# dmjovan/NeRF-Workspaces-Explorer

Hardware: AMD Instinct MI355X
Metric: ray-samples/sec (800x800, 192 samples, 8x256 MLP) (higher is better)
Workload: dtype f16x3 (split-fp16 MFMA, fp32 accumulate)

## Files before the change

### nerf-workspaces-explorer_amd/csrc/nwe_mfma_kernels.h

```cpp
#pragma once
#include "nwe_host.h"

namespace nwe {

typedef _Float16 h8 __attribute__((ext_vector_type(8)));
typedef float f16v __attribute__((ext_vector_type(16)));

#define LDS_AS __attribute__((address_space(3)))

constexpr int kWaves = 4;
constexpr int kRaysPerWave = 32;

template <int W, int D>
struct Shape {
    static constexpr int NT = W / 32;
    static constexpr int KH = W / 16;
    static constexpr int KG = 4;
    static constexpr int KD = 2;
    static constexpr int NTV = W / 64;
    static constexpr int KV = W / 32;
    static constexpr int N_L0 = 2 * KG / kWaves;
    static constexpr int N_H = 2 * KH / kWaves;
    static constexpr int N_S = 2 * (KH + KG) / kWaves;
    static constexpr int N_V = 2 * (KH + KD) / kWaves;
    static constexpr int N_RGB = 2 * KV / kWaves;
    static constexpr int CHUNK_BYTES = N_S * kWaves * kTileBytes;
    static constexpr int N_CHUNKS = NT + D * NT + 1 + NTV + 1;
    static constexpr int N_CHUNKS_FOLDED = N_CHUNKS - NT - 1;
    static constexpr int N_DOT_ROWS = NT + 1;
    static constexpr int N_CHUNKS_NOVIEW = D * NT + 1;
    static constexpr int n_chunks(int form) { return form == kFormFolded ? N_CHUNKS_FOLDED : (form == kFormNoViewDirs ? N_CHUNKS_NOVIEW : N_CHUNKS); }
    static constexpr int n_bias_rows(int form) { return n_chunks(form) + (form == kFormFolded ? N_DOT_ROWS : 0); }
    static constexpr int LONG_PIECES = 8;
};

struct Pend {
    f16v a;
    float4 bias[4];
};

__device__ __forceinline__ float pend_value(const Pend& t, int r, float inv_scale) {
    const float4 b = t.bias[r >> 2];
    const float bb = (r & 3) == 0 ? b.x : ((r & 3) == 1 ? b.y : ((r & 3) == 2 ? b.z : b.w));
    return __builtin_fmaf(t.a[r], inv_scale, bb);
}

typedef _Float16 h2 __attribute__((ext_vector_type(2)));

template <bool X3, bool DOT = false>
__device__ __forceinline__ void finish_elem(const Pend& t, int e, float inv_scale, float lower, float& keep, h8& hi0, h8& lo0,
                                            h8& hi1, h8& lo1, const float* dotw = nullptr, float* dot = nullptr) {
    const float v = fmaxf(pend_value(t, e, inv_scale), lower);
    if (DOT) *dot = __builtin_fmaf(dotw[8 * (e >> 2) + (e & 3)], v, *dot);
    if ((e & 1) == 0) { keep = v; return; }
    const float v0 = keep, v1 = v;
    h2 hp;
    hp[0] = (_Float16)v0; hp[1] = (_Float16)v1;
    const _Float16 h0 = hp[0], h1 = hp[1];
    _Float16 l0 = (_Float16)0.f, l1 = (_Float16)0.f;
    if (X3) {
        const uint32_t hw = __builtin_bit_cast(uint32_t, hp);
        float r0, r1;
        asm("v_fma_mix_f32 %0, %1, -1.0, %2 op_sel:[0,0,0] op_sel_hi:[1,0,0]" : "=v"(r0) : "v"(hw), "v"(v0));
        asm("v_fma_mix_f32 %0, %1, -1.0, %2 op_sel:[1,0,0] op_sel_hi:[1,0,0]" : "=v"(r1) : "v"(hw), "v"(v1));
        l0 = (_Float16)r0; l1 = (_Float16)r1;
    }
    if (e < 8) { hi0[e - 1] = h0; hi0[e] = h1; lo0[e - 1] = l0; lo0[e] = l1; }
    else { hi1[e - 9] = h0; hi1[e - 8] = h1; lo1[e - 9] = l0; lo1[e - 8] = l1; }
}

struct Epi {
    float v[16];
    float r[16];
    uint32_t hp[8];
    uint32_t lp[8];
    float dw[16];
};

template <bool X3, int NKH, int NQ, bool FEEDS, uint32_t PM>
struct EpiPlan {
    static constexpr int GPK = X3 ? 3 : 1;
    static constexpr int NS = X3 ? 8 : 5;
    static constexpr int NGAPS = GPK * NQ;
    static constexpr int D0 = FEEDS ? GPK * (NKH - 2) - 1 : NGAPS - 1;
    static constexpr int D1 = FEEDS ? GPK * (NKH - 1) - 1 : NGAPS - 1;
    static constexpr bool usable(int gi) { return gi >= 1 && gi < NGAPS && !(X3 && gi % GPK == 1 && ((PM >> (gi / GPK)) & 1u)); }
    static constexpr int gap_of(int n) {
        int c = -1;
        for (int gi = 0; gi < NGAPS; ++gi)
            if (usable(gi) && ++c == n) return gi;
        return 1 << 20;
    }
    static constexpr bool fits(int ng) { return gap_of((ng >= 2 ? ng / 2 : 1) * NS - 1) <= D0 && gap_of(ng * NS - 1) <= D1; }
    static constexpr int NG = fits(4) ? 4 : (fits(2) ? 2 : (fits(1) ? 1 : 0));
    static constexpr bool STAGED = NG > 0;
    static constexpr int GS = STAGED ? 16 / NG : 16;
    static constexpr int slot_at(int gi) {
        if (!usable(gi)) return -1;
        int c = 0;
        for (int g = 0; g < gi; ++g) c += usable(g) ? 1 : 0;
        return c < NG * NS ? c : -1;
    }
};

__device__ __forceinline__ h8 pack4(uint32_t a, uint32_t b, uint32_t c, uint32_t d) {
    typedef uint32_t u4 __attribute__((ext_vector_type(4)));
    u4 t = {a, b, c, d};
    return __builtin_bit_cast(h8, t);
}

template <class P, bool X3, int G, int ST, bool DOT>
__device__ __forceinline__ void epi_stage(const Pend& t, Epi& E, float inv_scale, float lower, h8& y0h, h8& y0l, h8& y1h, h8& y1l,
                                          const float* dotw, float& dot) {
    constexpr int st = ST, e0 = G * P::GS;
    constexpr int ST_PACK = 3, ST_RES = 4, ST_PACKLO = 5, ST_PARK = X3 ? 6 : 4;
    if constexpr (DOT) {
        static_assert(P::NS - ST_PACK >= 1, "no stage left for the dot product");
        constexpr int NDS = P::NS - ST_PACK;
        if (st == 1) {
#pragma unroll
            for (int q = e0 / 4; q < (e0 + P::GS) / 4; ++q) {
                const float4 w4 = *reinterpret_cast<const float4*>(dotw + 8 * q);
                E.dw[4 * q] = w4.x; E.dw[4 * q + 1] = w4.y; E.dw[4 * q + 2] = w4.z; E.dw[4 * q + 3] = w4.w;
            }
        }
        if (st >= ST_PACK) {
#pragma unroll
            for (int e = e0; e < e0 + P::GS; ++e)
                if ((e - e0) % NDS == st - ST_PACK) {
                    dot = __builtin_fmaf(E.dw[e], E.v[e], dot);
                    asm volatile("" : "+v"(dot));
                }
        }
    }
    if (st == 0) {
#pragma unroll
        for (int e = e0; e < e0 + P::GS; ++e) {
            float a = t.a[e];
            asm volatile("" : "+v"(a));
            E.v[e] = a;
        }
    } else if (st == 1) {
#pragma unroll
        for (int e = e0; e < e0 + P::GS; ++e) {
            const float4 b = t.bias[e >> 2];
            const float bb = (e & 3) == 0 ? b.x : ((e & 3) == 1 ? b.y : ((e & 3) == 2 ? b.z : b.w));
            E.v[e] = __builtin_fmaf(E.v[e], inv_scale, bb);
        }
    } else if (st == 2) {
#pragma unroll
        for (int e = e0; e < e0 + P::GS; ++e) E.v[e] = fmaxf(E.v[e], lower);
    } else if (st == ST_PACK) {
#pragma unroll
        for (int p = e0 / 2; p < (e0 + P::GS) / 2; ++p) {
            h2 hp;
            hp[0] = (_Float16)E.v[2 * p]; hp[1] = (_Float16)E.v[2 * p + 1];
            E.hp[p] = __builtin_bit_cast(uint32_t, hp);
            if (!X3) E.lp[p] = 0u;
        }
    } else if (X3 && st == ST_RES) {
#pragma unroll
        for (int p = e0 / 2; p < (e0 + P::GS) / 2; ++p) {
            asm("v_fma_mix_f32 %0, %1, -1.0, %2 op_sel:[0,0,0] op_sel_hi:[1,0,0]" : "=v"(E.r[2 * p]) : "v"(E.hp[p]), "v"(E.v[2 * p]));
            asm("v_fma_mix_f32 %0, %1, -1.0, %2 op_sel:[1,0,0] op_sel_hi:[1,0,0]" : "=v"(E.r[2 * p + 1]) : "v"(E.hp[p]), "v"(E.v[2 * p + 1]));
        }
    } else if (X3 && st == ST_PACKLO) {
#pragma unroll
        for (int p = e0 / 2; p < (e0 + P::GS) / 2; ++p) {
            h2 lp;
            lp[0] = (_Float16)E.r[2 * p]; lp[1] = (_Float16)E.r[2 * p + 1];
            E.lp[p] = __builtin_bit_cast(uint32_t, lp);
        }
    } else if (st == ST_PARK || st == ST_PARK + 1) {
        const bool lo = st != ST_PARK;
        if (lo && !X3) return;
        const int last = e0 + P::GS - 1;
        if (last == 7 || (P::GS == 16)) {
            if (!lo) { y0h = pack4(E.hp[0], E.hp[1], E.hp[2], E.hp[3]); asm volatile("" : "+a"(y0h)); }
            else     { y0l = pack4(E.lp[0], E.lp[1], E.lp[2], E.lp[3]); asm volatile("" : "+a"(y0l)); }
        }
        if (last == 15) {
            if (!lo) { y1h = pack4(E.hp[4], E.hp[5], E.hp[6], E.hp[7]); asm volatile("" : "+a"(y1h)); }
            else     { y1l = pack4(E.lp[4], E.lp[5], E.lp[6], E.lp[7]); asm volatile("" : "+a"(y1l)); }
        }
    }
}

template <class P, bool X3, int GI, bool DOT>
__device__ __forceinline__ void epi_gap(const Pend& t, Epi& E, float inv_scale, float lower, h8& y0h, h8& y0l, h8& y1h, h8& y1l,
                                        const float* dotw, float& dot) {
    constexpr int slot = P::slot_at(GI);
    if constexpr (slot >= 0) epi_stage<P, X3, slot / P::NS, slot % P::NS, DOT>(t, E, inv_scale, lower, y0h, y0l, y1h, y1l, dotw, dot);
}

template <bool X3>
__device__ __forceinline__ void mma3(const h8& a_hi, const h8& a_lo, const h8& x_hi, const h8& x_lo, f16v& acc) {
    acc = __builtin_amdgcn_mfma_f32_32x32x16_f16(a_hi, x_hi, acc, 0, 0, 0);
    if (X3) {
        acc = __builtin_amdgcn_mfma_f32_32x32x16_f16(a_lo, x_hi, acc, 0, 0, 0);
        acc = __builtin_amdgcn_mfma_f32_32x32x16_f16(a_hi, x_lo, acc, 0, 0, 0);
    }
}

template <int CHUNK_BYTES, bool X3>
struct Walker {
    const uint8_t* stream;
    uint32_t next_tile;
    uint32_t lds_chunks;
    uint32_t lds_tail;
    const char* buf0;
    const char* tail0;
    int t3;
    uint32_t blk_dst_tail;
    int tail_first;
    const float* bias_tab;
    int chunk;
    int b;
    int wave;
    uint32_t lane_off;
    const uint8_t* blk_src;
    uint32_t blk_dst;
    bool skip_lo = false;
#ifdef NWE_STAMPS
    unsigned long long st_pre = 0, st_wait = 0, st_post = 0, st_t0 = 0;
#endif

    __device__ __forceinline__ void start(const uint8_t* s, const float* bias) {
        stream = s; bias_tab = bias; next_tile = 0; chunk = 0; b = 0; t3 = 0;
    }
    __device__ __forceinline__ const char* cur() const { return buf0 + b * CHUNK_BYTES; }
    __device__ __forceinline__ const char* next() const { return buf0 + (b ^ 1) * CHUNK_BYTES; }
    __device__ __forceinline__ const char* tail() const { return tail0 + t3 * (2 * kTileBytes); }
    __device__ __forceinline__ void begin(int n_per_wave, int buffer, int ahead) {
        blk_src = stream + ((size_t)next_tile + (size_t)wave * n_per_wave) * kTileBytes;
        blk_dst = lds_chunks + buffer * CHUNK_BYTES + wave * n_per_wave * kTileBytes;
        next_tile += n_per_wave * kWaves;
        skip_lo = !X3 && (n_per_wave & 1) == 0;
        if (X3) {
            int slot = t3 + ahead;
            slot = slot >= 3 ? slot - 3 : slot;
            const bool lng = n_per_wave >= 8;
            tail_first = (lng && wave == kWaves - 1) ? n_per_wave - 2 : (1 << 20);
            blk_dst_tail = lds_tail + slot * (2 * kTileBytes) - (n_per_wave - 2) * kTileBytes;
        }
    }
    __device__ __forceinline__ void piece(int i, int tail_piece = -1) {
#ifdef NWE_EXP_NODMA
        return;
#endif
        if (!X3 && skip_lo && (i & 1)) return;
        const uint8_t* src = blk_src + (size_t)(i >> 2) * (4 * kTileBytes);
        const uint32_t base = (X3 && i >= 6 && i >= tail_first) ? blk_dst_tail : blk_dst;
        const uint32_t dst = base + (i >> 2) * (4 * kTileBytes);
        const bool set_m0 = (i & 3) == 0 || (X3 && i == tail_piece);
#ifndef NWE_GLDS_POLICY
#define NWE_GLDS_POLICY 0
#endif
#if NWE_GLDS_POLICY == 1
#define NWE_GLDS_POL " sc1"
#elif NWE_GLDS_POLICY == 2
#define NWE_GLDS_POL " nt"
#elif NWE_GLDS_POLICY == 3
#define NWE_GLDS_POL " sc0 sc1"
#elif NWE_GLDS_POLICY == 4
#define NWE_GLDS_POL " sc1 nt"
#else
#define NWE_GLDS_POL ""
#endif
#define NWE_GLDS(OFF) asm volatile("global_load_lds_dwordx4 %0, %1 offset:" #OFF NWE_GLDS_POL :: "v"(lane_off), "s"(src) : "memory")
#define NWE_GLDS_M0(OFF) asm volatile("s_mov_b32 m0, %2\n\ts_nop 0\n\tglobal_load_lds_dwordx4 %0, %1 offset:" #OFF NWE_GLDS_POL \
                                      :: "v"(lane_off), "s"(src), "s"(dst) : "memory")
        if (set_m0) {
            switch (i & 3) {
                case 0: NWE_GLDS_M0(0); break;
                case 1: NWE_GLDS_M0(1024); break;
                case 2: NWE_GLDS_M0(2048); break;
                default: NWE_GLDS_M0(3072); break;
            }
        } else {
            switch (i & 3) {
                case 1: NWE_GLDS(1024); break;
                case 2: NWE_GLDS(2048); break;
                default: NWE_GLDS(3072); break;
            }
        }
#undef NWE_GLDS
#undef NWE_GLDS_M0
// ... 64 lines not shown
    constexpr int NQ = NKH + NKD;
    constexpr int QSYNC = NQ - PD;
    static_assert(QSYNC >= 0, "tile too short for the prefetch distance");
    static_assert(NKP % R == 0, "the optional segment must not shift the fragment ring");
    const float4* bp = reinterpret_cast<const float4*>(wk.bias_tab + wk.chunk * 32);
    const int h = lane >> 5;
#ifndef NWE_SPREAD_BIAS
#define NWE_SPREAD_BIAS 1
#endif
    constexpr bool SPREAD_BIAS = X3 && NWE_SPREAD_BIAS != 0 && (NKH + NKD) >= 6;
    if constexpr (!SPREAD_BIAS) {
#pragma unroll
        for (int g = 0; g < 4; ++g) cur.bias[g] = bp[2 * g + h];
        __builtin_amdgcn_sched_group_barrier(0x100, 4, 0);
    }
    constexpr bool LONG_TILE = X3 && NQ >= 16;
    constexpr int S_LONG_PIECES = 8;
    const char* cbase = wk.cur() + lane * 16;
    const char* nbase = wk.next() + lane * 16;
    const char* tbase = wk.tail() + lane * 16;
    bool pre_done = false;
    float ekeep = 0.f;
    Epi E;
    if (NKP > 0) {
        if (use_g) {
#pragma unroll
            for (int s = 0; s < NKP; ++s) {
                const int slot = (PHASE + s + PD) % R;
                F.hi[slot] = *reinterpret_cast<const h8*>(cbase + (2 * (s + PD)) * kTileBytes);
                if (X3) F.lo[slot] = *reinterpret_cast<const h8*>(cbase + (2 * (s + PD) + 1) * kTileBytes);
                const int use = (PHASE + s) % R;
                if (s == 0) {
                    f16v zero;
#pragma unroll
                    for (int r = 0; r < 16; ++r) zero[r] = 0.f;
                    cur.a = __builtin_amdgcn_mfma_f32_32x32x16_f16(F.hi[use], Ghi[0], zero, 0, 0, 0);
                    if (X3) {
                        cur.a = __builtin_amdgcn_mfma_f32_32x32x16_f16(F.lo[use], Ghi[0], cur.a, 0, 0, 0);
                        cur.a = __builtin_amdgcn_mfma_f32_32x32x16_f16(F.hi[use], Glo[0], cur.a, 0, 0, 0);
                    }
                } else {
                    mma3<X3>(F.hi[use], F.lo[use], Ghi[s], Glo[s], cur.a);
                }
                __builtin_amdgcn_sched_group_barrier(0x100, X3 ? 2 : 1, 0);
                __builtin_amdgcn_sched_group_barrier(0x008, X3 ? 3 : 1, 0);
                __builtin_amdgcn_sched_barrier(0);
            }
            cbase += NKP * 2 * kTileBytes;
            pre_done = true;
        }
    }
    static_for<0, NQ>([&](auto qc) __attribute__((always_inline)) {
        constexpr int q = decltype(qc)::value;
        const h8* Xh = q < NKH ? &Xhi[q] : &Dhi[q - NKH];
        const h8* Xl = q < NKH ? &Xlo[q] : &Dlo[q - NKH];
        if (q == QSYNC) {
#ifdef NWE_STAMPS
            { const unsigned long long t = __builtin_amdgcn_s_memtime(); wk.st_pre += t - wk.st_t0; wk.st_t0 = t; }
#endif
            wk.template sync<LONG_TILE>();
#ifdef NWE_STAMPS
            { const unsigned long long t = __builtin_amdgcn_s_memtime(); wk.st_wait += t - wk.st_t0; wk.st_t0 = t; }
#endif
            if (NA > 0) wk.begin(na_override >= 0 ? na_override : NA + (extraA ? 2 : 0), wk.b, 2);
        }
        const int use = (PHASE + q) % R;
#ifndef NWE_ONE_WAIT
#define NWE_ONE_WAIT 1
#endif
        if constexpr (X3 && NWE_ONE_WAIT != 0) asm volatile("" :: "v"(F.hi[use]), "v"(F.lo[use]));
        if (q == 0 && !(NKP > 0 && pre_done)) {
            f16v zero;
#pragma unroll
            for (int r = 0; r < 16; ++r) zero[r] = 0.f;
            cur.a = __builtin_amdgcn_mfma_f32_32x32x16_f16(F.hi[use], *Xh, zero, 0, 0, 0);
        } else {
            cur.a = __builtin_amdgcn_mfma_f32_32x32x16_f16(F.hi[use], *Xh, cur.a, 0, 0, 0);
        }
        auto dma = [&]() __attribute__((always_inline)) {
            using DP = DmaPlan<NB, NA, NQ>;
            if constexpr (q < QSYNC && DP::TOT > 0) {
#pragma unroll
                for (int j = DP::lo(q); j < DP::lo(q + 1); ++j) {
                    if (j < DP::REST) wk.piece(PD + j, NB >= S_LONG_PIECES ? NB - 2 : -1);
                    else if (extraB) wk.piece(NB + j - DP::REST);
                }
            }
            if constexpr (q >= QSYNC && NA > 0 && q - QSYNC < (NA < PD ? NA : PD)) wk.piece(q - QSYNC);
        };
        if constexpr (!X3) dma();
#ifndef NWE_SPLIT_READS
#define NWE_SPLIT_READS 1
#endif
        auto read_frag = [&](bool want_hi, bool want_lo) __attribute__((always_inline)) {
            if (LONG_TILE && q + PD == NQ - 1) {
                const int slot = (PHASE + q + PD) % R;
                if (want_lo) F.lo[slot] = *reinterpret_cast<const h8*>(tbase + kTileBytes);
                if (want_hi) F.hi[slot] = *reinterpret_cast<const h8*>(tbase);
            } else if (q + PD < NQ) {
                const int slot = (PHASE + q + PD) % R;
                if (X3 && want_lo) F.lo[slot] = *reinterpret_cast<const h8*>(cbase + (2 * (q + PD) + 1) * kTileBytes);
                if (want_hi) F.hi[slot] = *reinterpret_cast<const h8*>(cbase + (2 * (q + PD)) * kTileBytes);
            } else if (HASNEXT) {
                const int slot = (PHASE + q + PD) % R;
                if (X3 && want_lo) F.lo[slot] = *reinterpret_cast<const h8*>(nbase + (2 * (q + PD - NQ) + 1) * kTileBytes);
                if (want_hi) F.hi[slot] = *reinterpret_cast<const h8*>(nbase + (2 * (q + PD - NQ)) * kTileBytes);
            }
        };
        constexpr bool SPLIT_RD = X3 && NWE_SPLIT_READS != 0;
        read_frag(true, !SPLIT_RD);
        using Plan = EpiPlan<X3, NKH, NQ, FEEDS, DmaPlan<NB, NA, NQ>::mask()>;
        constexpr int GPK = Plan::GPK;
#ifdef NWE_EXP_NOEPI
        if constexpr (PEND && q == 0) asm volatile("" :: "a"(prev.a));
#define NWE_EPI_ON false
#else
#define NWE_EPI_ON true
#endif
        if constexpr (NWE_EPI_ON && PEND && Plan::STAGED) epi_gap<Plan, X3, GPK * q, DOT>(prev, E, inv_scale, lower, y0h, y0l, y1h, y1l, dotw, dot_ref);
        if (NWE_EPI_ON && PEND && !Plan::STAGED && q < NKH) {
#pragma unroll
            for (int e = 0; e < 16; ++e)
                if ((e * (NKH - 1)) / 16 == q) {
                    finish_elem<X3, DOT>(prev, e, inv_scale, lower, ekeep, y0h, y0l, y1h, y1l, dotw, &dot_ref);
                    if (e == 7) asm volatile("" : "+a"(y0h), "+a"(y0l));
                }
        }
        __builtin_amdgcn_sched_group_barrier(0x008, 1, 0);
        if (q + PD < NQ || HASNEXT) __builtin_amdgcn_sched_group_barrier(0x100, (X3 && !SPLIT_RD) ? 2 : 1, 0);
        if (X3) {
            __builtin_amdgcn_sched_barrier(0);
            cur.a = __builtin_amdgcn_mfma_f32_32x32x16_f16(F.lo[use], *Xh, cur.a, 0, 0, 0);
            dma();
            if constexpr (NWE_EPI_ON && PEND && Plan::STAGED) epi_gap<Plan, X3, GPK * q + 1, DOT>(prev, E, inv_scale, lower, y0h, y0l, y1h, y1l, dotw, dot_ref);
            __builtin_amdgcn_sched_group_barrier(0x008, 1, 0);
            __builtin_amdgcn_sched_barrier(0);
            cur.a = __builtin_amdgcn_mfma_f32_32x32x16_f16(F.hi[use], *Xl, cur.a, 0, 0, 0);
            if constexpr (SPLIT_RD) read_frag(false, true);
            if constexpr (SPREAD_BIAS && q >= 1 && q <= 4) cur.bias[q - 1] = bp[2 * (q - 1) + h];
            if constexpr (NWE_EPI_ON && PEND && Plan::STAGED) epi_gap<Plan, X3, GPK * q + 2, DOT>(prev, E, inv_scale, lower, y0h, y0l, y1h, y1l, dotw, dot_ref);
            __builtin_amdgcn_sched_group_barrier(0x008, 1, 0);
            if (SPLIT_RD && (q + PD < NQ || HASNEXT)) __builtin_amdgcn_sched_group_barrier(0x100, 1, 0);
            if (SPREAD_BIAS && q >= 1 && q <= 4) __builtin_amdgcn_sched_group_barrier(0x100, 1, 0);
        }
        __builtin_amdgcn_sched_barrier(0);
    });
    if (PEND) asm volatile("" : "+a"(y1h), "+a"(y1l));
#ifdef NWE_STAMPS
    { const unsigned long long t = __builtin_amdgcn_s_memtime(); wk.st_post += t - wk.st_t0; wk.st_t0 = t; }
#endif
    wk.tile_done();
}

template <int NT, int NKP, int NKH, bool X3, bool PEND0, int N_AFTER, bool PASS_START, bool DOT = false, int NA_LAST = N_AFTER, class WalkerT>
__device__ __forceinline__ void layer(WalkerT& wk, Frags& F, int lane, bool use_g, bool extra_after, const h8* Ghi, const h8* Glo,
                                      h8* Xhi, h8* Xlo, h8* Yhi, h8* Ylo, Pend& P0, Pend& P1, float inv_scale, float lower_prev,
                                      float lower, int na_last_override = -1, const float* dot_tab = nullptr, float* dot = nullptr) {
    static_assert(NT % 2 == 0 && NT >= 4, "tiles per layer must be even (accumulator ping-pong)");
    constexpr int N_THIS = 2 * NKH / kWaves;
#pragma unroll
    for (int rt = 0; rt < NT; ++rt) {
        Pend& cur = (rt & 1) ? P1 : P0;
        Pend& prev = (rt & 1) ? P0 : P1;
        const bool ebB = rt + 1 < NT ? use_g : extra_after;
        const bool ebA = rt + 2 < NT ? use_g : extra_after;
        const float* drow = DOT ? dot_tab + (rt - 1) * 32 : nullptr;
        if (rt == 0) {
            constexpr int NB0 = PASS_START ? 0 : N_THIS;
            if constexpr (PEND0) {
                constexpr int L = 2 * NT - 2;
                tile_mma<NKP, NKH, 0, 0, X3, true, NB0, N_THIS, true, true>(wk, F, lane, use_g, ebB, ebA, Ghi, Glo, Xhi, Xlo, nullptr, nullptr,
                                                                      cur, prev, inv_scale, lower_prev, Xhi[L], Xlo[L], Xhi[L + 1], Xlo[L + 1]);
            } else {
                h8 d0, d1, d2, d3;
                tile_mma<NKP, NKH, 0, 0, X3, false, NB0, N_THIS, true>(wk, F, lane, use_g, ebB, ebA, Ghi, Glo, Xhi, Xlo, nullptr, nullptr,
                                                                       cur, prev, inv_scale, lower_prev, d0, d1, d2, d3);
            }
        } else if (rt + 2 < NT) {
            tile_mma<NKP, NKH, 0, 0, X3, true, N_THIS, N_THIS, true, false, DOT>(wk, F, lane, use_g, ebB, ebA, Ghi, Glo, Xhi, Xlo, nullptr, nullptr, cur,
                                                                     prev, inv_scale, lower, Yhi[2 * rt - 2], Ylo[2 * rt - 2], Yhi[2 * rt - 1],
                                                                     Ylo[2 * rt - 1], -1, drow, dot);
        } else if (rt + 1 < NT) {
            tile_mma<NKP, NKH, 0, 0, X3, true, N_THIS, N_AFTER, true, false, DOT>(wk, F, lane, use_g, ebB, ebA, Ghi, Glo, Xhi, Xlo, nullptr, nullptr, cur,
                                                                      prev, inv_scale, lower, Yhi[2 * rt - 2], Ylo[2 * rt - 2], Yhi[2 * rt - 1],
                                                                      Ylo[2 * rt - 1], -1, drow, dot);
        } else {
            tile_mma<NKP, NKH, 0, 0, X3, true, N_AFTER, NA_LAST, true, false, DOT>(wk, F, lane, use_g, ebB, ebA, Ghi, Glo, Xhi, Xlo, nullptr, nullptr, cur,
                                                                       prev, inv_scale, lower, Yhi[2 * rt - 2], Ylo[2 * rt - 2], Yhi[2 * rt - 1],
                                                                       Ylo[2 * rt - 1], na_last_override, drow, dot);
        }
    }
}

template <int NB, int NK, bool X3>
__device__ __forceinline__ void encode(float vx, float vy, float vz, int h, h8* Ehi, h8* Elo) {
    float vals[NK * 8];
#pragma unroll
    for (int i = 0; i < NK * 8; ++i) vals[i] = 0.f;
    const float first = h ? (float)(1 << NB) : 1.f;
#pragma unroll
    for (int c = 0; c < 3; ++c) {
        const float v = c == 0 ? vx : (c == 1 ? vy : vz);
        float sn[NB], cs[NB];
        octave_sincos<NB>(v, first, sn, cs);
#pragma unroll
        for (int bl = 0; bl < NB; ++bl) {
            vals[2 * (bl * 3 + c)] = sn[bl];
            vals[2 * (bl * 3 + c) + 1] = cs[bl];
        }
    }
    vals[6 * NB] = h ? vz : vx;
    vals[6 * NB + 1] = h ? 0.f : vy;
#pragma unroll
    for (int s = 0; s < NK; ++s) {
#pragma unroll
        for (int j = 0; j < 8; ++j) {
            const float v = vals[s * 8 + j];
            const _Float16 hh = (_Float16)v;
            Ehi[s][j] = hh;
            Elo[s][j] = X3 ? (_Float16)(v - (float)hh) : (_Float16)0.f;
        }
    }
}

template <int RT, int W, int D, bool X3, bool SIGMA_TILE, class WalkerT>
__device__ __forceinline__ void view_tiles(WalkerT& wk, Frags& F, int lane, h8* Ahi, h8* Alo, const h8* GDhi,
                                           const h8* GDlo, h8* Bhi, h8* Blo, Pend& P0, Pend& P1, float inv_scale,
                                           const float* dot_tab = nullptr, float* dot = nullptr) {
    using S = Shape<W, D>;
    constexpr int par = SIGMA_TILE ? (RT + 1) & 1 : RT & 1;
    Pend& cur = par ? P1 : P0;
    Pend& prev = par ? P0 : P1;
    constexpr int PH = (RT * (S::KH + S::KD)) % (PD + 1);
    constexpr int NB = RT + 1 < S::NTV ? S::N_V : S::N_RGB;
    constexpr int NA = RT + 2 < S::NTV ? S::N_V : (RT + 2 == S::NTV ? S::N_RGB : 0);
    if constexpr (RT == 0 && SIGMA_TILE) {
        h8 d0, d1, d2, d3;
        tile_mma<0, S::KH, S::KD, PH, X3, false, NB, NA, true>(wk, F, lane, false, false, false, nullptr, nullptr, Ahi, Alo, GDhi, GDlo, cur,
                                                               prev, inv_scale, 0.f, d0, d1, d2, d3);
    } else if constexpr (RT == 0) {
        constexpr int L = 2 * S::NT - 2;
        tile_mma<0, S::KH, S::KD, PH, X3, true, NB, NA, true, true, true>(wk, F, lane, false, false, false, nullptr, nullptr, Ahi, Alo, GDhi, GDlo,
                                                                          cur, prev, inv_scale, 0.f, Ahi[L], Alo[L], Ahi[L + 1], Alo[L + 1], -1,
                                                                          dot_tab + (S::NT - 1) * 32, dot);
    } else {
        tile_mma<0, S::KH, S::KD, PH, X3, true, NB, NA, true>(wk, F, lane, false, false, false, nullptr, nullptr, Ahi, Alo, GDhi, GDlo, cur,
                                                              prev, inv_scale, 0.f, Bhi[2 * RT - 2], Blo[2 * RT - 2], Bhi[2 * RT - 1],
                                                              Blo[2 * RT - 1]);
    }
    if constexpr (RT + 1 < S::NTV) view_tiles<RT + 1, W, D, X3, SIGMA_TILE>(wk, F, lane, Ahi, Alo, GDhi, GDlo, Bhi, Blo, P0, P1, inv_scale);
}

template <int W, int D, int SKIP, bool X3, int FORM, class WalkerT>
__device__ __forceinline__ void mlp_eval(WalkerT& wk, Frags& F, int lane, float inv_scale, h8* Ghi, h8* Glo, const char* gd_lds,
                                         const float* dot_tab, float& o_r, float& o_g, float& o_b, float& o_s) {
    using S = Shape<W, D>;
    static_assert(D % 2 == 0, "trunk depth must be even");
    static_assert(SKIP < 0 || SKIP % 2 == 0, "skip layer index must be even");
    static_assert(S::NT % 2 == 0 && S::NTV % 2 == 0, "tile counts must be even");
    constexpr bool FOLD = FORM == kFormFolded, NOVIEW = FORM == kFormNoViewDirs;
    h8 Ahi[S::KH], Alo[S::KH], Bhi[S::KH], Blo[S::KH];
    Pend P0, P1;
    constexpr int NPAIR = D / 2;
    constexpr int SKIP_PAIR = SKIP < 0 ? -1 : SKIP / 2;

    layer<S::NT, 0, S::KG, X3, false, S::N_H, true>(wk, F, lane, false, SKIP_PAIR == 0, nullptr, nullptr, Ghi, Glo, Ahi, Alo, P0, P1,
                                                    inv_scale, 0.f, 0.f);
    auto pair_body = [&](bool use_g, bool skip_next, bool last) __attribute__((always_inline)) {
        layer<S::NT, S::KG, S::KH, X3, true, S::N_H, false>(wk, F, lane, use_g, false, Ghi, Glo, Ahi, Alo, Bhi, Blo, P0, P1, inv_scale,
                                                            0.f, 0.f);
        layer<S::NT, 0, S::KH, X3, true, S::N_H, false>(wk, F, lane, false, skip_next, nullptr, nullptr, Bhi, Blo,
                                                        Ahi, Alo, P0, P1, inv_scale, 0.f, (FORM == kFormReference && last) ? -INFINITY : 0.f,
                                                        (FORM == kFormReference && last) ? S::N_V : -1);
    };
    constexpr int PAIRS = FORM == kFormReference ? NPAIR : NPAIR - 1;
#ifndef NWE_PEEL_SKIP
#define NWE_PEEL_SKIP 1
#endif
    if constexpr (NWE_PEEL_SKIP != 0 && SKIP_PAIR >= 0 && SKIP_PAIR < PAIRS) {
#pragma unroll 1
        for (int pair = 0; pair < SKIP_PAIR; ++pair) pair_body(false, pair + 1 == SKIP_PAIR, false);
        pair_body(true, false, SKIP_PAIR == NPAIR - 1);
#pragma unroll 1
        for (int pair = SKIP_PAIR + 1; pair < PAIRS; ++pair) pair_body(false, false, pair == NPAIR - 1);
    } else {
#pragma unroll 1
        for (int pair = 0; pair < PAIRS; ++pair) {
            const bool last = pair == NPAIR - 1;
            pair_body(pair == SKIP_PAIR, !last && pair + 1 == SKIP_PAIR, last);
        }
    }
    float sig = 0.f;
    if constexpr (FOLD) {
        constexpr bool G_LAST = SKIP_PAIR == NPAIR - 1;
        layer<S::NT, G_LAST ? S::KG : 0, S::KH, X3, true, S::N_V, false, true>(wk, F, lane, G_LAST, false, Ghi, Glo, Ahi, Alo, Bhi, Blo, P0, P1,
                                                                               inv_scale, 0.f, 0.f, -1, dot_tab, &sig);
    }
    constexpr int L = 2 * S::NT - 2;
    constexpr int LV = 2 * S::NTV - 2;
    if constexpr (NOVIEW) {
        constexpr bool G_LAST = SKIP_PAIR == NPAIR - 1;
        layer<S::NT, G_LAST ? S::KG : 0, S::KH, X3, true, S::N_H, false, false, 0>(wk, F, lane, G_LAST, false, Ghi, Glo, Ahi, Alo, Bhi, Blo, P0, P1,
                                                                                   inv_scale, 0.f, 0.f);
        tile_mma<0, S::KH, 0, 0, X3, true, 0, 0, false, true>(wk, F, lane, false, false, false, nullptr, nullptr, Bhi, Blo, nullptr, nullptr, P0,
                                                              P1, inv_scale, 0.f, Bhi[L], Blo[L], Bhi[L + 1], Blo[L + 1]);
        o_r = pend_value(P0, 0, inv_scale);
        o_g = pend_value(P0, 1, inv_scale);
        o_b = pend_value(P0, 2, inv_scale);
        o_s = pend_value(P0, 3, inv_scale);
        return;
    }
    static_assert((S::NTV * (S::KH + S::KD)) % (PD + 1) == 0, "the view tiles must restore the ring phase");
    h8 GDhi[S::KD], GDlo[S::KD];
#pragma unroll
    for (int k = 0; k < S::KD; ++k) {
        GDhi[k] = *reinterpret_cast<const h8*>(gd_lds + (2 * k) * kTileBytes);
        if (X3) GDlo[k] = *reinterpret_cast<const h8*>(gd_lds + (2 * k + 1) * kTileBytes);
    }
    if constexpr (FOLD) {
        view_tiles<0, W, D, X3, false>(wk, F, lane, Bhi, Blo, GDhi, GDlo, Ahi, Alo, P0, P1, inv_scale, dot_tab, &sig);
        const float sigma = __fadd_rn(__fadd_rn(sig, __shfl_xor(sig, 32, 64)), dot_tab[S::NT * 32]);
        tile_mma<0, S::KV, 0, 0, X3, true, 0, 0, false, true>(wk, F, lane, false, false, false, nullptr, nullptr, Ahi, Alo, nullptr, nullptr, P0,
                                                              P1, inv_scale, 0.f, Ahi[LV], Alo[LV], Ahi[LV + 1], Alo[LV + 1]);
        o_s = sigma;
        o_r = pend_value(P0, 0, inv_scale);
        o_g = pend_value(P0, 1, inv_scale);
        o_b = pend_value(P0, 2, inv_scale);
        return;
    } else {
        tile_mma<0, S::KH, 0, 0, X3, true, S::N_V, S::N_V, true>(wk, F, lane, false, false, false, nullptr, nullptr, Bhi, Blo, nullptr, nullptr,
                                                                 P0, P1, inv_scale, -INFINITY, Ahi[L], Alo[L], Ahi[L + 1], Alo[L + 1]);
        const float sigma = pend_value(P0, 0, inv_scale);
        view_tiles<0, W, D, X3, true>(wk, F, lane, Ahi, Alo, GDhi, GDlo, Bhi, Blo, P0, P1, inv_scale);
        tile_mma<0, S::KV, 0, 0, X3, true, 0, 0, false, true>(wk, F, lane, false, false, false, nullptr, nullptr, Bhi, Blo, nullptr, nullptr, P1,
                                                              P0, inv_scale, 0.f, Bhi[LV], Blo[LV], Bhi[LV + 1], Blo[LV + 1]);
        o_s = sigma;
    }
    o_r = pend_value(P1, 0, inv_scale);
    o_g = pend_value(P1, 1, inv_scale);
    o_b = pend_value(P1, 2, inv_scale);
}

constexpr int kPacketMaxSamples = 64;
constexpr int kSplitMaxSamples = kMaxSamples;

template <int W, int D, bool SPLIT>
struct Smem {
    using S = Shape<W, D>;
    static constexpr int WBYTES = (SPLIT ? kSplitMaxSamples : kWaves * kPacketMaxSamples) * kRaysPerWave * 4;
    static constexpr int CHUNKS = 2 * S::CHUNK_BYTES;
    static constexpr int BOFF = CHUNKS;
    static constexpr int BIAS_BYTES = ((S::N_CHUNKS * 32 * 4 + 255) / 256) * 256;
    static constexpr int WOFF = BOFF + 2 * BIAS_BYTES;
    static constexpr int TOFF = WOFF + WBYTES;
    static constexpr int XOFF = TOFF + (2 * kMaxSamples + kMaxImportance) * 4;
    static constexpr int LOFF = XOFF + (SPLIT ? 2 * kWaves * kRaysPerWave * 16 : 0);
    static constexpr int GOFF = LOFF + 3 * 2 * kTileBytes;
    static constexpr int TOTAL = GOFF + kWaves * 2 * S::KD * kTileBytes;
    static_assert(XOFF % 16 == 0 && LOFF % 16 == 0 && GOFF % 16 == 0 && TOTAL <= 160 * 1024, "LDS budget");
};

__host__ __device__ inline bool is_lean(const RenderArgs& a) {
    const nwe_outputs& o = a.out;
    return !o.raw_coarse && !o.raw_fine && !o.z_fine && !o.weights_coarse && !o.disp && !o.z_std && !o.rgb_coarse && !o.depth_coarse &&
           !o.acc_coarse && !o.disp_coarse && !o.sample_cond && !o.sample_amp && !o.sample_switch && !o.feat_map && !a.z_fine_in && !a.raw_in_c &&
           !a.raw_in_f && !a.w_in && !a.t_rand && !a.noise_c && !a.noise_f && !a.u_rand && !a.stamps && !a.rays;
}

template <int W, int D, int SKIP, bool X3, bool SPLIT, int FORM, bool LEAN>
__global__ void __launch_bounds__(256) render_mfma_kernel(RenderArgs a_in, NetMfma nc, NetMfma nf) {
    RenderArgs a = a_in;
    if constexpr (LEAN) {
        a.out.raw_coarse = a.out.raw_fine = a.out.z_fine = a.out.weights_coarse = nullptr;
        a.out.disp = a.out.z_std = a.out.rgb_coarse = a.out.depth_coarse = a.out.acc_coarse = a.out.disp_coarse = nullptr;
        a.out.sample_cond = a.out.sample_amp = a.out.sample_switch = a.out.feat_map = nullptr;
        a.z_fine_in = a.raw_in_c = a.raw_in_f = a.w_in = a.t_rand = a.noise_c = a.noise_f = a.u_rand = nullptr;
        a.stamps = nullptr; a.rays = nullptr;
    }
    using S = Shape<W, D>;
    using SM = Smem<W, D, SPLIT>;
    __shared__ __attribute__((aligned(16))) char smem[SM::TOTAL];

    const int lane = threadIdx.x & 63;
    const int wave = __builtin_amdgcn_readfirstlane(threadIdx.x >> 6);
    const int half = lane >> 5;
    const int ns = a.n_samples, ni = a.n_importance;

    float* s_t = reinterpret_cast<float*>(smem + SM::TOFF);
    float* s_omt = s_t + kMaxSamples;
    float* s_u = s_omt + kMaxSamples;
    for (int i = threadIdx.x; i < ns; i += 256) { s_t[i] = a.t_vals[i]; s_omt[i] = a.omt_vals[i]; }
    for (int i = threadIdx.x; i < ni; i += 256) s_u[i] = a.u_vals[i];
    float* s_bias = reinterpret_cast<float*>(smem + SM::BOFF);
    constexpr int NCH = S::n_chunks(FORM);
    constexpr int NROWS = S::n_bias_rows(FORM);
    static_assert(NROWS * 32 * 4 <= SM::BIAS_BYTES, "bias table too small for the dot rows");
    for (int i = threadIdx.x; i < NROWS * 32; i += 256) {
        s_bias[i] = nc.bias[i];
        if (ni > 0) s_bias[SM::BIAS_BYTES / 4 + i] = nf.bias[i];
    }

    const int64_t packet = SPLIT ? (int64_t)blockIdx.x : (int64_t)blockIdx.x * kWaves + wave;
    const int64_t ridx64 = a.ray_first + packet * kRaysPerWave + (lane & 31);
    const bool lane_live = ridx64 < a.n_rays && half == 0;
    const bool live = lane_live && (!SPLIT || wave == 0);
    const int row = (int)(ridx64 < a.n_rays ? ridx64 : a.n_rays - 1);
    const int64_t ridx = row, rclamp = row;
    const RaySeed seed = seed_ray(a, rclamp);
    auto fresh_ray = [&]() __attribute__((always_inline)) {
        RaySeed sd = seed;
        asm volatile("" : "+v"(sd.pose), "+v"(sd.x), "+v"(sd.y));
        return make_ray<false>(a, sd);
    };

    Walker<S::CHUNK_BYTES, X3> wk;
    wk.buf0 = smem; wk.lds_chunks = (uint32_t)(uintptr_t)(LDS_AS char*)smem;
    wk.tail0 = smem + SM::LOFF; wk.lds_tail = wk.lds_chunks + SM::LOFF; wk.t3 = 0;
    wk.b = 0; wk.wave = wave; wk.lane_off = lane * 16;

    char* gd_lds = smem + SM::GOFF + wave * (2 * S::KD * kTileBytes) + lane * 16;
    if constexpr (FORM != kFormNoViewDirs) {
        const Ray rv = make_ray<true>(a, seed);
        h8 GDhi[S::KD], GDlo[S::KD];
        encode<2, S::KD, X3>(rv.vx, rv.vy, rv.vz, half, GDhi, GDlo);
#pragma unroll
        for (int k = 0; k < S::KD; ++k) {
            *reinterpret_cast<h8*>(gd_lds + (2 * k) * kTileBytes) = GDhi[k];
            *reinterpret_cast<h8*>(gd_lds + (2 * k + 1) * kTileBytes) = GDlo[k];
        }
    }

    FineSampler fs;
    fs.wc = reinterpret_cast<float*>(smem + SM::WOFF) + (SPLIT ? 0 : wave * (kPacketMaxSamples * kRaysPerWave)) + (lane & 31);
    const bool wc_writer = !SPLIT || wave == 0;
    fs.stride = kRaysPerWave; fs.u_tab = s_u; fs.ns = ns; fs.ni = ni;
    fs.cd.t_tab = s_t; fs.cd.omt_tab = s_omt; fs.cd.ns = ns;
    fs.cd.jitter = a.t_rand; fs.cd.row = row;
    fs.u_rand = a.u_rand;
    __syncthreads();

    Composite comp;
    uint32_t flags = 0;
#ifdef NWE_STAMPS
    unsigned long long st_enc = 0, st_sync = 0, st_mlp = 0, st_comp = 0;
    const unsigned long long st_begin = __builtin_amdgcn_s_memtime();
    const unsigned long long st_real = __builtin_amdgcn_s_memrealtime();
#endif
    for (int pass = 0; pass < (ni > 0 ? 2 : 1); ++pass) {
        const NetMfma& net = pass == 0 ? nc : nf;
        const float* bias = s_bias + (pass == 0 ? 0 : SM::BIAS_BYTES / 4);
        const float* dot_tab = bias + NCH * 32;
        const int Stot = pass == 0 ? ns : ns + ni;
        const float* noise = pass == 0 ? a.noise_c : a.noise_f;
        const float* raw_in = pass == 0 ? a.raw_in_c : a.raw_in_f;
        if (pass == 0 && a.w_in) {
            if (wc_writer) for (int s = 0; s < ns; ++s) fs.wc[s * kRaysPerWave] = a.w_in[rclamp * ns + s];
            continue;
        }
        comp.reset();
        if constexpr (SPLIT) {
            int produced = 0;
            auto gen = [&](const Ray& ray) -> float {
                const int i = produced++;
                if (i >= Stot) return 0.f;
                if (pass == 0) return fs.cd.z(ray, i);
                return a.z_fine_in ? a.z_fine_in[rclamp * Stot + i] : fs.next(ray);
            };
            float zq[5], zp[4];
            {
                const Ray ray = fresh_ray();
                if (pass == 1) {
                    if (wc_writer) fs.build_cdf();
                    __syncthreads();
                    fs.start(ray);
                    if (wants_survey(a.out)) {
                        const SampleSurvey sv = fs.survey(ray);
                        if (live) flags |= store_survey(a.out, ridx, sv);
                    }
                }
#pragma unroll
                for (int k = 0; k < 5; ++k) zq[k] = gen(ray);
            }
            float4* xch = reinterpret_cast<float4*>(smem + SM::XOFF);
            const int n_it = (Stot + 3) / 4;
            auto drain = [&](int it) {
                const float4* x = xch + (it & 1) * (kWaves * kRaysPerWave) + (lane & 31);
#pragma unroll
                for (int k = 0; k < 4; ++k) {
                    const int si = 4 * it + k;
                    if (si < Stot) {
                        const float w = comp.accumulate(x[k * kRaysPerWave], zp[k]);
                        if (pass == 0) {
                            if (wc_writer) fs.wc[si * kRaysPerWave] = w;
                            if (live && a.out.weights_coarse) a.out.weights_coarse[ridx * ns + si] = w;
                        }
                    }
                }
            };
            for (int it = 0; it < n_it; ++it) {
#ifdef NWE_STAMPS
                const unsigned long long t0 = __builtin_amdgcn_s_memtime();
#endif
                if (!raw_in) {
                    wk.start(net.stream, bias);
                    wk.begin(S::N_L0, 0, 0);
#pragma unroll
                    for (int i = 0; i < S::N_L0; ++i) wk.piece(i);
                    wk.begin(S::N_L0, 1, 1);
#pragma unroll
                    for (int i = 0; i < S::N_L0; ++i) wk.piece(i);
                }
                const Ray ray = fresh_ray();
                const int s_own = 4 * it + wave;
                const bool own_valid = s_own < Stot;
                float z_own = zq[0], z_nxt = zq[1];
                if (wave == 1) { z_own = zq[1]; z_nxt = zq[2]; }
                if (wave == 2) { z_own = zq[2]; z_nxt = zq[3]; }
                if (wave == 3) { z_own = zq[3]; z_nxt = zq[4]; }
                float nz[4];
#pragma unroll
                for (int k = 0; k < 4; ++k) nz[k] = gen(ray);
                float rr, rg, rb, rs;
                if (raw_in) {
                    __syncthreads();
                    if (it > 0) drain(it - 1);
#pragma unroll
                    for (int k = 0; k < 4; ++k) zp[k] = zq[k];
                    const float4 v = *reinterpret_cast<const float4*>(raw_in + (rclamp * Stot + (own_valid ? s_own : Stot - 1)) * 4);
                    rr = v.x; rg = v.y; rb = v.z; rs = v.w;
                } else {
                float px, py, pz;
                point_at(ray, z_own, px, py, pz);
                h8 Ghi[S::KG], Glo[S::KG];
                encode<5, S::KG, X3>(__fdiv_rn(px, 10.f), __fdiv_rn(py, 10.f), __fdiv_rn(pz, 10.f), half, Ghi, Glo);
#ifdef NWE_STAMPS
                const unsigned long long t1 = __builtin_amdgcn_s_memtime();
                st_enc += t1 - t0;
#endif
                wk.template sync<false>();
                Frags F;
#pragma unroll
                for (int k = 0; k < PD; ++k) {
                    F.hi[k] = *reinterpret_cast<const h8*>(wk.cur() + lane * 16 + (2 * k) * kTileBytes);
                    if (X3) F.lo[k] = *reinterpret_cast<const h8*>(wk.cur() + lane * 16 + (2 * k + 1) * kTileBytes);
                }
                if (it > 0) drain(it - 1);
#pragma unroll
                for (int k = 0; k < 4; ++k) zp[k] = zq[k];
#ifdef NWE_STAMPS
                const unsigned long long t2 = __builtin_amdgcn_s_memtime();
                wk.st_t0 = t2;
                st_sync += t2 - t1;
#endif
                mlp_eval<W, D, SKIP, X3, FORM>(wk, F, lane, net.inv_scale, Ghi, Glo, gd_lds, dot_tab, rr, rg, rb, rs);
#ifdef NWE_STAMPS
                st_mlp += __builtin_amdgcn_s_memtime() - t2;
#endif
                }
#ifdef NWE_STAMPS
                const unsigned long long t3 = __builtin_amdgcn_s_memtime();
#endif
                if (own_valid) {
                    xch[(it & 1) * (kWaves * kRaysPerWave) + wave * kRaysPerWave + (lane & 31)] =
                        Composite::shade(rr, rg, rb, rs, z_own, z_nxt, s_own + 1 == Stot, ray.dnorm, noise ? noise[rclamp * Stot + s_own] : 0.f);
                    if (lane_live) {
                        float* raw = pass == 0 ? a.out.raw_coarse : a.out.raw_fine;
                        if (raw) {
                            *reinterpret_cast<float4*>(raw + (ridx * Stot + s_own) * 4) = make_float4(rr, rg, rb, rs);
                            if (bad(rr) || bad(rg) || bad(rb) || bad(rs)) flags |= NWE_FLAG_RAW;
                        }
                        if (pass == 1 && a.out.z_fine) a.out.z_fine[ridx * Stot + s_own] = z_own;
                    }
                }
                zq[0] = zq[4];
#pragma unroll
                for (int k = 0; k < 4; ++k) zq[k + 1] = nz[k];
#ifdef NWE_STAMPS
                st_comp += __builtin_amdgcn_s_memtime() - t3;
#endif
            }
            __syncthreads();
            drain(n_it - 1);
            __syncthreads();
        } else {
            float z_cur, z_next = 0.f;
            {
                const Ray ray = fresh_ray();
                if (pass == 0) z_cur = fs.cd.z(ray, 0);
                else {
                    fs.prepare(ray);
                    if (wants_survey(a.out)) {
                        const SampleSurvey sv = fs.survey(ray);
                        if (live) flags |= store_survey(a.out, ridx, sv);
                    }
                    z_cur = a.z_fine_in ? a.z_fine_in[rclamp * Stot] : fs.next(ray);
                }
            }
            for (int s = 0; s < Stot; ++s) {
    #ifdef NWE_STAMPS
                const unsigned long long t0 = __builtin_amdgcn_s_memtime();
    #endif
                if (!raw_in) {
                    wk.start(net.stream, bias);
                    wk.begin(S::N_L0, 0, 0);
    #pragma unroll
                    for (int i = 0; i < S::N_L0; ++i) wk.piece(i);
                    wk.begin(S::N_L0, 1, 1);
    #pragma unroll
                    for (int i = 0; i < S::N_L0; ++i) wk.piece(i);
                }
                const Ray ray = fresh_ray();
                if (s + 1 < Stot) {
                    if (pass == 0) z_next = fs.cd.z(ray, s + 1);
                    else z_next = a.z_fine_in ? a.z_fine_in[rclamp * Stot + s + 1] : fs.next(ray);
                }
                float rr, rg, rb, rs;
                if (raw_in) {
                    const float4 v = *reinterpret_cast<const float4*>(raw_in + (rclamp * Stot + s) * 4);
                    rr = v.x; rg = v.y; rb = v.z; rs = v.w;
                } else {
                float px, py, pz;
                point_at(ray, z_cur, px, py, pz);
                h8 Ghi[S::KG], Glo[S::KG];
                encode<5, S::KG, X3>(__fdiv_rn(px, 10.f), __fdiv_rn(py, 10.f), __fdiv_rn(pz, 10.f), half, Ghi, Glo);
    #ifdef NWE_STAMPS
                const unsigned long long t1 = __builtin_amdgcn_s_memtime();
                st_enc += t1 - t0;
    #endif
                wk.template sync<false>();
                Frags F;
    #pragma unroll
                for (int k = 0; k < PD; ++k) {
                    F.hi[k] = *reinterpret_cast<const h8*>(wk.cur() + lane * 16 + (2 * k) * kTileBytes);
                    if (X3) F.lo[k] = *reinterpret_cast<const h8*>(wk.cur() + lane * 16 + (2 * k + 1) * kTileBytes);
                }
    #ifdef NWE_STAMPS
                const unsigned long long t2 = __builtin_amdgcn_s_memtime();
                wk.st_t0 = t2;
                st_sync += t2 - t1;
    #endif
                mlp_eval<W, D, SKIP, X3, FORM>(wk, F, lane, net.inv_scale, Ghi, Glo, gd_lds, dot_tab, rr, rg, rb, rs);
    #ifdef NWE_STAMPS
                st_mlp += __builtin_amdgcn_s_memtime() - t2;
    #endif
                }
    #ifdef NWE_STAMPS
                const unsigned long long t3 = __builtin_amdgcn_s_memtime();
    #endif
                const float w = comp.step(rr, rg, rb, rs, z_cur, z_next, s + 1 == Stot, ray.dnorm, noise ? noise[rclamp * Stot + s] : 0.f);
                if (pass == 0) fs.wc[s * kRaysPerWave] = w;
                if (lane_live) {
                    if (pass == 0 && a.out.weights_coarse) a.out.weights_coarse[ridx * ns + s] = w;
                    float* raw = pass == 0 ? a.out.raw_coarse : a.out.raw_fine;
                    if (raw) {
                        *reinterpret_cast<float4*>(raw + (ridx * Stot + s) * 4) = make_float4(rr, rg, rb, rs);
                        if (bad(rr) || bad(rg) || bad(rb) || bad(rs)) flags |= NWE_FLAG_RAW;
                    }
                    if (pass == 1 && a.out.z_fine) a.out.z_fine[ridx * Stot + s] = z_cur;
                }
                z_cur = z_next;
    #ifdef NWE_STAMPS
                st_comp += __builtin_amdgcn_s_memtime() - t3;
    #endif
            }
        }
        if (live) {
            flags |= store_ray(a.out, ridx, comp, pass == 1, a.white_bkgd != 0);
            if (ni == 0) flags |= store_ray(a.out, ridx, comp, true, a.white_bkgd != 0);
        }
    }
    if (flags && a.out.flags) atomicOr(a.out.flags, flags);
#ifdef NWE_STAMPS
    if (a.stamps && lane == 0) {
        unsigned long long* o = a.stamps + ((size_t)blockIdx.x * kWaves + wave) * 10;
        o[0] = st_enc; o[1] = st_sync; o[2] = st_mlp; o[3] = st_comp; o[4] = __builtin_amdgcn_s_memtime() - st_begin;
        o[5] = wk.st_pre; o[6] = wk.st_wait; o[7] = wk.st_post;
        o[8] = __builtin_amdgcn_s_memrealtime() - st_real; o[9] = st_begin;
    }
#endif
}

template <int W, int D, int SKIP, int FORM>
inline void launch_one(RenderArgs a, const NetMfma& nc, const NetMfma& nf, bool three_pass, bool split, int64_t ray_first, int64_t rays,
                       hipStream_t stream) {
    if (rays <= 0) return;
    a.ray_first = ray_first;
    const int64_t per_wg = split ? kRaysPerWave : kWaves * kRaysPerWave;
    const unsigned blocks = (unsigned)((rays + per_wg - 1) / per_wg);
#define NWE_LAUNCH(X3_, SPLIT_, LEAN_) \
    hipLaunchKernelGGL((render_mfma_kernel<W, D, SKIP, X3_, SPLIT_, FORM, LEAN_>), dim3(blocks), dim3(256), 0, stream, a, nc, nf)
    const bool lean = is_lean(a);
    if (three_pass) {
        if (split) { if (lean) NWE_LAUNCH(true, true, true); else NWE_LAUNCH(true, true, false); }
        else       { if (lean) NWE_LAUNCH(true, false, true); else NWE_LAUNCH(true, false, false); }
    } else {
        if (split) { if (lean) NWE_LAUNCH(false, true, true); else NWE_LAUNCH(false, true, false); }
        else       { if (lean) NWE_LAUNCH(false, false, true); else NWE_LAUNCH(false, false, false); }
    }
#undef NWE_LAUNCH
}

template <int W, int D, int SKIP, int FORM>
bool launch_t(const RenderArgs& a, const NetMfma& nc, const NetMfma& nf, bool three_pass, int decomposition, hipStream_t stream,
                     LaunchInfo* info) {
    using S = Shape<W, D>;
    constexpr int NCH = S::n_chunks(FORM);
    if (nc.n_chunks != NCH || (a.n_importance > 0 && nf.n_chunks != NCH)) return false;
    int dev = 0, cus = 256;
    if (hipGetDevice(&dev) == hipSuccess) (void)hipDeviceGetAttribute(&cus, hipDeviceAttributeMultiprocessorCount, dev);
    if (cus <= 0) cus = 256;
    const int64_t rays_wg = kWaves * kRaysPerWave;
    const double its = (double)(a.n_samples + (a.n_importance > 0 ? a.n_samples + a.n_importance : 0));
    const double its_split = 1.06 * (double)((a.n_samples + 3) / 4 + (a.n_importance > 0 ? (a.n_samples + a.n_importance + 3) / 4 : 0));
    const auto rounds = [&](int64_t rays, int64_t per_wg) { return (double)(((rays + per_wg - 1) / per_wg + cus - 1) / cus); };
    const int64_t full = (a.n_rays / rays_wg / cus) * cus * rays_wg;
    const double t_packet = rounds(a.n_rays, rays_wg) * its;
    const double t_split = rounds(a.n_rays, kRaysPerWave) * its_split;
    const double t_hybrid = full > 0 && full < a.n_rays ? (double)(full / rays_wg / cus) * its + rounds(a.n_rays - full, kRaysPerWave) * its_split : 1e300;
    const double t_single = t_packet <= t_split ? t_packet : t_split;
    int plan = t_hybrid < 0.992 * t_single ? 2 : (t_packet <= t_split ? 0 : 1);
    if (decomposition >= 0) plan = decomposition;
    if (a.n_samples > kPacketMaxSamples) plan = 1;
    if (info) { info->plan = plan; info->rays_first = plan == 2 ? full : a.n_rays; info->mid_recorded = false; }
    if (plan == 2) {
        launch_one<W, D, SKIP, FORM>(a, nc, nf, three_pass, false, 0, full, stream);
        if (info && info->mid) info->mid_recorded = hipEventRecord(info->mid, stream) == hipSuccess;
        launch_one<W, D, SKIP, FORM>(a, nc, nf, three_pass, true, full, a.n_rays - full, stream);
    } else {
        launch_one<W, D, SKIP, FORM>(a, nc, nf, three_pass, plan == 1, 0, a.n_rays, stream);
    }
    return true;
}


}
```

Baseline: 335.7 million.

## Skip view-direction branch in coarse pass when only density is needed

Adds a density-only path for the coarse pass of a hierarchical render. When fine samples follow, it evaluates only the trunk and the sigma dot product, then skips the view-direction and RGB tiles. The last trunk layer's DMA plan is adjusted so nothing is streamed for the view tiles, and a drain step finishes the dot on the pending accumulator. The coarse RGB output becomes zero and its flag is masked, which changes what the coarse outputs contain. That is a risk if callers expect coarse RGB.

```diff
diff --git a/nerf-workspaces-explorer_amd/csrc/nwe_mfma_kernels.h b/nerf-workspaces-explorer_amd/csrc/nwe_mfma_kernels.h
--- a/nerf-workspaces-explorer_amd/csrc/nwe_mfma_kernels.h
+++ b/nerf-workspaces-explorer_amd/csrc/nwe_mfma_kernels.h
@@ -109,11 +109,12 @@
     return __builtin_bit_cast(h8, t);
 }
 
-template <class P, bool X3, int G, int ST, bool DOT>
+template <class P, bool X3, int G, int ST, bool DOT, bool ACT = true>
 __device__ __forceinline__ void epi_stage(const Pend& t, Epi& E, float inv_scale, float lower, h8& y0h, h8& y0l, h8& y1h, h8& y1l,
                                           const float* dotw, float& dot) {
     constexpr int st = ST, e0 = G * P::GS;
     constexpr int ST_PACK = 3, ST_RES = 4, ST_PACKLO = 5, ST_PARK = X3 ? 6 : 4;
+    static_assert(ACT || DOT, "a stage without activation output only serves the dot product");
     if constexpr (DOT) {
         static_assert(P::NS - ST_PACK >= 1, "no stage left for the dot product");
         constexpr int NDS = P::NS - ST_PACK;
@@ -133,6 +134,7 @@
                 }
         }
     }
+    if constexpr (!ACT && st >= ST_PACK) return;
     if (st == 0) {
 #pragma unroll
         for (int e = e0; e < e0 + P::GS; ++e) {
@@ -503,11 +505,28 @@
     wk.tile_done();
 }
 
-template <int NT, int NKP, int NKH, bool X3, bool PEND0, int N_AFTER, bool PASS_START, bool DOT = false, int NA_LAST = N_AFTER, class WalkerT>
+template <class P, bool X3>
+__device__ __forceinline__ void drain_dot(const Pend& t, float inv_scale, const float* dotw, float& dot) {
+    if constexpr (P::STAGED) {
+        Epi E;
+        h8 d0, d1, d2, d3;
+        static_for<0, P::NG * P::NS>([&](auto sc) __attribute__((always_inline)) {
+            constexpr int s = decltype(sc)::value;
+            epi_stage<P, X3, s / P::NS, s % P::NS, true, false>(t, E, inv_scale, 0.f, d0, d1, d2, d3, dotw, dot);
+        });
+    } else {
+#pragma unroll
+        for (int e = 0; e < 16; ++e) dot = __builtin_fmaf(dotw[8 * (e >> 2) + (e & 3)], fmaxf(pend_value(t, e, inv_scale), 0.f), dot);
+    }
+}
+
+template <int NT, int NKP, int NKH, bool X3, bool PEND0, int N_AFTER, bool PASS_START, bool DOT = false, int NA_LAST = N_AFTER,
+          bool LAST_HASNEXT = true, class WalkerT>
 __device__ __forceinline__ void layer(WalkerT& wk, Frags& F, int lane, bool use_g, bool extra_after, const h8* Ghi, const h8* Glo,
                                       h8* Xhi, h8* Xlo, h8* Yhi, h8* Ylo, Pend& P0, Pend& P1, float inv_scale, float lower_prev,
                                       float lower, int na_last_override = -1, const float* dot_tab = nullptr, float* dot = nullptr) {
     static_assert(NT % 2 == 0 && NT >= 4, "tiles per layer must be even (accumulator ping-pong)");
+    static_assert(LAST_HASNEXT || (N_AFTER == 0 && NA_LAST == 0), "a layer that ends the evaluation streams nothing behind it");
     constexpr int N_THIS = 2 * NKH / kWaves;
 #pragma unroll
     for (int rt = 0; rt < NT; ++rt) {
@@ -536,7 +555,7 @@
                                                                       prev, inv_scale, lower, Yhi[2 * rt - 2], Ylo[2 * rt - 2], Yhi[2 * rt - 1],
                                                                       Ylo[2 * rt - 1], -1, drow, dot);
         } else {
-            tile_mma<NKP, NKH, 0, 0, X3, true, N_AFTER, NA_LAST, true, false, DOT>(wk, F, lane, use_g, ebB, ebA, Ghi, Glo, Xhi, Xlo, nullptr, nullptr, cur,
+            tile_mma<NKP, NKH, 0, 0, X3, true, N_AFTER, NA_LAST, LAST_HASNEXT, false, DOT>(wk, F, lane, use_g, ebB, ebA, Ghi, Glo, Xhi, Xlo, nullptr, nullptr, cur,
                                                                        prev, inv_scale, lower, Yhi[2 * rt - 2], Ylo[2 * rt - 2], Yhi[2 * rt - 1],
                                                                        Ylo[2 * rt - 1], na_last_override, drow, dot);
         }
@@ -573,6 +592,14 @@
         }
     }
 }
+
+template <int W, int D, bool X3>
+struct ViewDma {
+    using S = Shape<W, D>;
+    static constexpr int nb(int rt) { return rt + 1 < S::NTV ? S::N_V : S::N_RGB; }
+    static constexpr int na(int rt) { return rt + 2 < S::NTV ? S::N_V : (rt + 2 == S::NTV ? S::N_RGB : 0); }
+    using Plan0 = EpiPlan<X3, S::KH, S::KH + S::KD, true, DmaPlan<nb(0), na(0), S::KH + S::KD>::mask()>;
+};
 
 template <int RT, int W, int D, bool X3, bool SIGMA_TILE, class WalkerT>
 __device__ __forceinline__ void view_tiles(WalkerT& wk, Frags& F, int lane, h8* Ahi, h8* Alo, const h8* GDhi,
@@ -583,8 +610,8 @@
     Pend& cur = par ? P1 : P0;
     Pend& prev = par ? P0 : P1;
     constexpr int PH = (RT * (S::KH + S::KD)) % (PD + 1);
-    constexpr int NB = RT + 1 < S::NTV ? S::N_V : S::N_RGB;
-    constexpr int NA = RT + 2 < S::NTV ? S::N_V : (RT + 2 == S::NTV ? S::N_RGB : 0);
+    constexpr int NB = ViewDma<W, D, X3>::nb(RT);
+    constexpr int NA = ViewDma<W, D, X3>::na(RT);
     if constexpr (RT == 0 && SIGMA_TILE) {
         h8 d0, d1, d2, d3;
         tile_mma<0, S::KH, S::KD, PH, X3, false, NB, NA, true>(wk, F, lane, false, false, false, nullptr, nullptr, Ahi, Alo, GDhi, GDlo, cur,
@@ -602,9 +629,17 @@
     if constexpr (RT + 1 < S::NTV) view_tiles<RT + 1, W, D, X3, SIGMA_TILE>(wk, F, lane, Ahi, Alo, GDhi, GDlo, Bhi, Blo, P0, P1, inv_scale);
 }
 
+#ifndef NWE_COARSE_DENSITY_ONLY
+#define NWE_COARSE_DENSITY_ONLY 1
+#endif
+template <int D, int SKIP>
+constexpr bool density_only_built(int form) {
+    return NWE_COARSE_DENSITY_ONLY != 0 && form == kFormFolded && !(SKIP >= 0 && SKIP / 2 == D / 2 - 1);
+}
+
 template <int W, int D, int SKIP, bool X3, int FORM, class WalkerT>
 __device__ __forceinline__ void mlp_eval(WalkerT& wk, Frags& F, int lane, float inv_scale, h8* Ghi, h8* Glo, const char* gd_lds,
-                                         const float* dot_tab, float& o_r, float& o_g, float& o_b, float& o_s) {
+                                         const float* dot_tab, bool density_only, float& o_r, float& o_g, float& o_b, float& o_s) {
     using S = Shape<W, D>;
     static_assert(D % 2 == 0, "trunk depth must be even");
     static_assert(SKIP < 0 || SKIP % 2 == 0, "skip layer index must be even");
@@ -642,8 +677,26 @@
         }
     }
     float sig = 0.f;
+    auto sigma_of = [&]() __attribute__((always_inline)) { return __fadd_rn(__fadd_rn(sig, __shfl_xor(sig, 32, 64)), dot_tab[S::NT * 32]); };
     if constexpr (FOLD) {
         constexpr bool G_LAST = SKIP_PAIR == NPAIR - 1;
+        if constexpr (density_only_built<D, SKIP>(FORM)) {
+            if (density_only) {
+                using TrunkA = EpiPlan<X3, S::KH, S::KH, false, DmaPlan<S::N_H, S::N_V, S::KH>::mask()>;
+                using TrunkA0 = EpiPlan<X3, S::KH, S::KH, false, DmaPlan<S::N_H, 0, S::KH>::mask()>;
+                using TrunkB = EpiPlan<X3, S::KH, S::KH, false, DmaPlan<S::N_V, S::N_V, S::KH>::mask()>;
+                using TrunkB0 = EpiPlan<X3, S::KH, S::KH, false, DmaPlan<0, 0, S::KH>::mask()>;
+                static_assert(TrunkA::NG == TrunkA0::NG && TrunkB::NG == TrunkB0::NG,
+                              "the last trunk tiles must run the epilogues they carry in the full evaluation's order (dot FMAs)");
+                static_assert(!G_LAST, "density_only_built: the last trunk layer takes no gamma(x) k-steps here");
+                layer<S::NT, 0, S::KH, X3, true, 0, false, true, 0, false>(wk, F, lane, false, false, nullptr, nullptr, Ahi, Alo, Bhi, Blo, P0, P1,
+                                                                           inv_scale, 0.f, 0.f, -1, dot_tab, &sig);
+                drain_dot<typename ViewDma<W, D, X3>::Plan0, X3>(P1, inv_scale, dot_tab + (S::NT - 1) * 32 + 4 * (lane >> 5), sig);
+                o_s = sigma_of();
+                o_r = o_g = o_b = 0.f;
+                return;
+            }
+        }
         layer<S::NT, G_LAST ? S::KG : 0, S::KH, X3, true, S::N_V, false, true>(wk, F, lane, G_LAST, false, Ghi, Glo, Ahi, Alo, Bhi, Blo, P0, P1,
                                                                                inv_scale, 0.f, 0.f, -1, dot_tab, &sig);
     }
@@ -670,7 +723,7 @@
     }
     if constexpr (FOLD) {
         view_tiles<0, W, D, X3, false>(wk, F, lane, Bhi, Blo, GDhi, GDlo, Ahi, Alo, P0, P1, inv_scale, dot_tab, &sig);
-        const float sigma = __fadd_rn(__fadd_rn(sig, __shfl_xor(sig, 32, 64)), dot_tab[S::NT * 32]);
+        const float sigma = sigma_of();
         tile_mma<0, S::KV, 0, 0, X3, true, 0, 0, false, true>(wk, F, lane, false, false, false, nullptr, nullptr, Ahi, Alo, nullptr, nullptr, P0,
                                                               P1, inv_scale, 0.f, Ahi[LV], Alo[LV], Ahi[LV + 1], Alo[LV + 1]);
         o_s = sigma;
@@ -802,6 +855,7 @@
         const float* bias = s_bias + (pass == 0 ? 0 : SM::BIAS_BYTES / 4);
         const float* dot_tab = bias + NCH * 32;
         const int Stot = pass == 0 ? ns : ns + ni;
+        const bool density_only = LEAN && density_only_built<D, SKIP>(FORM) && pass == 0 && ni > 0;
         const float* noise = pass == 0 ? a.noise_c : a.noise_f;
         const float* raw_in = pass == 0 ? a.raw_in_c : a.raw_in_f;
         if (pass == 0 && a.w_in) {
@@ -903,7 +957,7 @@
                 wk.st_t0 = t2;
                 st_sync += t2 - t1;
 #endif
-                mlp_eval<W, D, SKIP, X3, FORM>(wk, F, lane, net.inv_scale, Ghi, Glo, gd_lds, dot_tab, rr, rg, rb, rs);
+                mlp_eval<W, D, SKIP, X3, FORM>(wk, F, lane, net.inv_scale, Ghi, Glo, gd_lds, dot_tab, density_only, rr, rg, rb, rs);
 #ifdef NWE_STAMPS
                 st_mlp += __builtin_amdgcn_s_memtime() - t2;
 #endif
@@ -990,7 +1044,7 @@
                 wk.st_t0 = t2;
                 st_sync += t2 - t1;
     #endif
-                mlp_eval<W, D, SKIP, X3, FORM>(wk, F, lane, net.inv_scale, Ghi, Glo, gd_lds, dot_tab, rr, rg, rb, rs);
+                mlp_eval<W, D, SKIP, X3, FORM>(wk, F, lane, net.inv_scale, Ghi, Glo, gd_lds, dot_tab, density_only, rr, rg, rb, rs);
     #ifdef NWE_STAMPS
                 st_mlp += __builtin_amdgcn_s_memtime() - t2;
     #endif
@@ -1016,7 +1070,7 @@
             }
         }
         if (live) {
-            flags |= store_ray(a.out, ridx, comp, pass == 1, a.white_bkgd != 0);
+            flags |= store_ray(a.out, ridx, comp, pass == 1, a.white_bkgd != 0) & (density_only ? ~(uint32_t)NWE_FLAG_RGB_COARSE : ~0u);
             if (ni == 0) flags |= store_ray(a.out, ridx, comp, true, a.white_bkgd != 0);
         }
     }
```

Result: faster. 340.7 million, median of 6 (+1.5%).
